# nzfeng/signed-heat-3d

Hardware: AMD Instinct MI355X
Metric: grid-nodes/sec end-to-end SHM (conv+PCG) (higher is better)
Workload: dtype f64 (Step 1: f64 / packed-f32 tiers)

## Files before the change

### signed-heat-3d_amd/csrc/shm_schur.hip.h

```cpp
#pragma once
#include "shm_kernels.hip.h"

namespace shm {

static __global__ __launch_bounds__(kBlock) void green_symbol_kernel(int n, const double* __restrict__ lam1, double* __restrict__ W0) {
    const double g0 = 0.5 / n, g1 = 1.0 / n;
    for (int row = blockIdx.x; row < n * n; row += gridDim.x) {
        const int k1 = row / n, k2 = row - k1 * n;
        const double l12 = lam1[k1] + lam1[k2];
        const double g12 = (k1 ? g1 : g0) * (k2 ? g1 : g0);
        double* const out = W0 + (size_t)row * n;
        for (int k3 = threadIdx.x; k3 < n; k3 += kBlock) {
            const double lam = l12 + lam1[k3];
            const double g = g12 * (k3 ? g1 : g0);
            out[k3] = (row | k3) ? g / lam : 0.;
        }
    }
}

static __global__ __launch_bounds__(kBlock) void cosine_tables_kernel(int n, int P, const double* __restrict__ ctab, double* __restrict__ Cm, double* __restrict__ Ct) {
    const int total = (n + 1) * n;
    for (int v = blockIdx.x * kBlock + threadIdx.x; v < total; v += gridDim.x * kBlock) {
        const int d = v / n, k = v - d * n;
        const double c = ctab[(int)(((long long)d * k) % (2 * n))];
        Cm[(size_t)d * n + k] = c;
        Ct[(size_t)k * P + d] = c;
    }
}

constexpr int kGemmT = 128, kGemmK = 16;
template <int WN>
__global__ __launch_bounds__(kBlock) __attribute__((amdgpu_waves_per_eu(WN == 4 ? 2 : WN == 2 ? 3 : 4, WN == 4 ? 2 : WN == 2 ? 3 : 4))) void dgemm_rm_kernel(int M, int N, int K, const double* __restrict__ A, int lda, long long sA, const double* __restrict__ B, int ldb,
                                                          long long sB, double* __restrict__ C, int ldc, long long sC, int prio) {
    constexpr int kTN = 32 * WN;
    if (prio) __builtin_amdgcn_s_setprio(3);
    __shared__ double as[kGemmT][kGemmK + 1];
    __shared__ double bs[kGemmK][kTN + 1];
    A += (long long)blockIdx.z * sA;
    B += (long long)blockIdx.z * sB;
    C += (long long)blockIdx.z * sC;
    const int i0 = blockIdx.y * kGemmT, j0 = blockIdx.x * kTN;
    const int lane = threadIdx.x & 63, w = threadIdx.x >> 6;
    const int wr = w >> 1, wc = w & 1;
    const int l15 = lane & 15, l4 = lane >> 4;
    gj_f64x4 acc[4][WN];
#pragma unroll
    for (int a = 0; a < 4; a++)
#pragma unroll
        for (int b = 0; b < WN; b++) acc[a][b] = gj_f64x4{0., 0., 0., 0.};
    constexpr int kPerA = kGemmT * kGemmK / kBlock, kPerB = kTN * kGemmK / kBlock;
    double ra[kPerA], rb[kPerB];
    auto fetch = [&](int kc) {
#pragma unroll
        for (int u = 0; u < kPerA; u++) {
            const int t = threadIdx.x + u * kBlock;
            const int k = t & (kGemmK - 1), i = t >> 4;
            ra[u] = (i0 + i < M && kc + k < K) ? A[(size_t)(i0 + i) * lda + kc + k] : 0.;
        }
#pragma unroll
        for (int u = 0; u < kPerB; u++) {
            const int t = threadIdx.x + u * kBlock;
            const int j = t & (kTN - 1), k2 = t / kTN;
            rb[u] = (kc + k2 < K && j0 + j < N) ? B[(size_t)(kc + k2) * ldb + j0 + j] : 0.;
        }
    };
    fetch(0);
    for (int kc = 0; kc < K; kc += kGemmK) {
        __syncthreads();
#pragma unroll
        for (int u = 0; u < kPerA; u++) {
            const int t = threadIdx.x + u * kBlock;
            as[t >> 4][t & (kGemmK - 1)] = ra[u];
        }
#pragma unroll
        for (int u = 0; u < kPerB; u++) {
            const int t = threadIdx.x + u * kBlock;
            bs[t / kTN][t & (kTN - 1)] = rb[u];
        }
        __syncthreads();
        if (kc + kGemmK < K) fetch(kc + kGemmK);
#pragma unroll
        for (int kk = 0; kk < kGemmK; kk += 4) {
            double af[4], bf[WN];
#pragma unroll
            for (int a = 0; a < 4; a++) af[a] = as[wr * 64 + a * 16 + l15][kk + l4];
#pragma unroll
            for (int b = 0; b < WN; b++) bf[b] = bs[kk + l4][wc * 16 * WN + b * 16 + l15];
#pragma unroll
            for (int a = 0; a < 4; a++)
#pragma unroll
                for (int b = 0; b < WN; b++) acc[a][b] = __builtin_amdgcn_mfma_f64_16x16x4f64(af[a], bf[b], acc[a][b], 0, 0, 0);
        }
    }
#pragma unroll
    for (int a = 0; a < 4; a++)
#pragma unroll
        for (int b = 0; b < WN; b++)
#pragma unroll
            for (int r = 0; r < 4; r++) {
                const int row = i0 + wr * 64 + a * 16 + l4 + 4 * r, col = j0 + wc * 16 * WN + b * 16 + l15;
                if (row < M && col < N) C[(size_t)row * ldc + col] = acc[a][b][r];
            }
}

__device__ __forceinline__ int schur_fold(int e, int n) { return e <= n ? e : 2 * n - e; }
typedef double schur_f64x2 __attribute__((ext_vector_type(2), aligned(8)));
static __global__ __launch_bounds__(kBlock) void schur_assemble_kernel(int m, int ld, int n, int P, const int* __restrict__ rowX ,
                                                                const double* __restrict__ rowT , const double* __restrict__ T, double* __restrict__ S, int prio) {
    if (blockIdx.x < blockIdx.y) return;
    if (prio) __builtin_amdgcn_s_setprio(3);
    const int i = blockIdx.y * 16 + (threadIdx.x >> 4), j = blockIdx.x * 16 + (threadIdx.x & 15);
    if (i >= m || j >= m || j < i) return;
    unsigned ox[2][3], oy[2][3], oz[2];
    double wx[2][3], wy[2][3], wz[2][3];
    const unsigned pitch_y = (unsigned)P, pitch_x = (unsigned)(n + 1) * (unsigned)P;
#pragma unroll
    for (int a = 0; a < 3; a++) {
        const int Xi = rowX[4 * i + a], Xj = rowX[4 * j + a];
        const double ti = rowT[3 * i + a], tj = rowT[3 * j + a];
        const double wi0 = 1. - ti, wi1 = ti, wj0 = 1. - tj, wj1 = tj;
        const int D = Xi - Xj, E = Xi + Xj + 1;
        const double wd[3] = {wi0 * wj1, wi0 * wj0 + wi1 * wj1, wi1 * wj0};
        const double ws[3] = {wi0 * wj0, wi0 * wj1 + wi1 * wj0, wi1 * wj1};
        int pd[3], ps[3];
#pragma unroll
        for (int e = 0; e < 3; e++) {
            pd[e] = abs(D - 1 + e);
            ps[e] = schur_fold(E + e, n);
        }
        if (a == 0) {
#pragma unroll
            for (int e = 0; e < 3; e++) {
                ox[0][e] = __umul24((unsigned)pd[e], pitch_x);
                ox[1][e] = __umul24((unsigned)ps[e], pitch_x);
                wx[0][e] = wd[e];
                wx[1][e] = ws[e];
            }
        } else if (a == 1) {
#pragma unroll
            for (int e = 0; e < 3; e++) {
                oy[0][e] = __umul24((unsigned)pd[e], pitch_y);
                oy[1][e] = __umul24((unsigned)ps[e], pitch_y);
                wy[0][e] = wd[e];
                wy[1][e] = ws[e];
            }
        } else {
#pragma unroll
            for (int f = 0; f < 2; f++) {
                const int* pz = f ? ps : pd;
                const double* wv = f ? ws : wd;
                const int zb = min(pz[0], min(pz[1], pz[2]));
                oz[f] = (unsigned)zb;
#pragma unroll
                for (int sl = 0; sl < 3; sl++) {
                    double w = 0.;
#pragma unroll
                    for (int e = 0; e < 3; e++) w += pz[e] - zb == sl ? wv[e] : 0.;
                    wz[f][sl] = w;
                }
            }
        }
    }
    double acc = 0.;
#pragma unroll
    for (int combo = 0; combo < 8; combo++) {
        const int fx = combo & 1, fy = (combo >> 1) & 1, fz = combo >> 2;
        const double* base = T + oz[fz];
        double sc = 0.;
#pragma unroll
        for (int p = 0; p < 3; p++) {
            double sp = 0.;
#pragma unroll
            for (int q = 0; q < 3; q++) {
                const double* row = base + (ox[fx][p] + oy[fy][q]);
                const schur_f64x2 lo = *reinterpret_cast<const schur_f64x2*>(row);
                const double hi = row[2];
                sp += wy[fy][q] * (wz[fz][0] * lo.x + wz[fz][1] * lo.y + wz[fz][2] * hi);
            }
            sc += wx[fx][p] * sp;
        }
        acc += sc;
    }
    const int ri = rowX[4 * i + 3], rj = rowX[4 * j + 3];
    S[(size_t)ri * ld + rj] = acc;
    S[(size_t)rj * ld + ri] = acc;
}

static __global__ __launch_bounds__(kBlock) void set_diagonal_kernel(double* __restrict__ M, int ld, int i0, int i1, double v) {
    const int i = i0 + blockIdx.x * kBlock + threadIdx.x;
    if (i < i1) M[(size_t)i * ld + i] = v;
}

static __global__ __launch_bounds__(kDualBlock) void dual_bordered_kernel(int m, const double* __restrict__ u, const double* __restrict__ v, const double* __restrict__ sigma_ptr,
                                                                  int accumulate, double* __restrict__ mu) {
    __shared__ double lds[17];
    double su = 0., sv = 0.;
    for (int a = threadIdx.x; a < m; a += kDualBlock) {
        su += u[a];
        sv += v[a];
    }
    su = block_sum_1024(su, lds);
    sv = block_sum_1024(sv, lds);
    const double c = (su - (sigma_ptr ? *sigma_ptr : 0.)) / sv;
    for (int a = threadIdx.x; a < m; a += kDualBlock) mu[a] = (accumulate ? mu[a] : 0.) + u[a] - c * v[a];
}

static __global__ __launch_bounds__(kBlock) void fill_kernel(double* __restrict__ x, int count, double v) {
    const int a = blockIdx.x * kBlock + threadIdx.x;
    if (a < count) x[a] = v;
}

}
```

### signed-heat-3d_amd/csrc/shm_solver.hip.h

```cpp
#pragma once
#include "shm_host.hip.h"
#include "shm_kernels.hip.h"
#include "shm_conv_tiered.hip.h"
#include "shm_cg_fused.hip.h"
#include "shm_twolevel.hip.h"
#include "shm_schur.hip.h"
#include "shm_dct.hip.h"
#include "shm_dct_gemm.hip.h"
#include "shm_green_fft.hip.h"
#include "shm_sample.hip.h"
#include "shm_audit.hip.h"
#include "shm_iso_indexed.hip.h"
#include "shm_plan.h"

namespace shm {

template <typename T> constexpr int vec_width() { return sizeof(T) == 8 ? 2 : 4; }

template <typename T>
struct Slab {
    int k0 = 0, k1 = 0, nzl = 0;
    size_t plane = 0, nown = 0, ntot = 0;
    DevArray<T> Y0, Y1, Y2, r , x, p, q , z ;
    DevArray<double> partials, pq_partials , red , pq , u , sc;
    DevArray<unsigned> proj_ticket;
    DevArray<int> row_ptr, ent_row, node_ptr;
    DevArray<uint32_t> ent_node, node_id;
    DevArray<double> ent_coef, nent_coef;
    DevArray<ShiftItem> shift_items;
    DevArray<double> dv;
    DevArray<int> layer_order;
    DevArray<int> sample_order;
    DevArray<unsigned char> sample_rule;
    DevArray<unsigned long long> sample_ctr;
    long long sample_key = -1;
    int sample_blocks = 0;
    long long layer_order_key = -1;
    DevArray<double> div_partials;
    int div_sum_blocks = 0;
    DevArray<T> touched_save;
    DevArray<T> W1, W2;
    DevArray<T> S1, S2, S4;
    DevArray<int> act_x, act_y;
    DevArray<unsigned> act_z;
    DevArray<int> act_planes;
    int n_act_planes = 0;
    int n_act_x = 0, n_act_y = 0;
    int n_touched = 0, n_shift = 0;
    GridParams gp{};
};

template <typename T>
struct Solver final : SolverBase {
    shm_config cfg;
    hipStream_t stream = nullptr;
    hipStream_t stream2 = nullptr;
    hipStream_t stream3 = nullptr;
    std::unique_ptr<Event> e_sch_in, e_sch_done, e_gs_done;
    hipStream_t stream_h = nullptr;
    int n = 0, alloc_n = -1;
    size_t N = 0;
    double cell = 0., lambda = 0.;
    double bbox_min[3] = {0, 0, 0};
    double conv_ctr[3] = {0, 0, 0};
    double conv_wscale = 1.;
    int64_t S = 0;
    std::vector<double> h_pos, h_wn, h_area;
    double area_sum = 0., conv_far_gap = 0., conv_skip_base = 3.0e38, last_host_setup_ms = 0., last_setup_wall_ms = 0.;
    double conv_tier_log = 0., conv_tier_skip_base = 3.0e38;
    double conv_drop_K = 64., conv_drop_eps64 = 2e-9, conv_drop_eps32 = 6.0e-8;
    double conv_w_span = 0.;
    DevArray<double> d_src_t;
    DevArray<float> d_clusters_t;
    int n_clusters_t = 0;
    bool conv_tiered = false;
    bool conv_tier_exact = false;
    bool conv_tiered32 = false;
    bool conv_reference = false;
    int step1_selected = SHM_STEP1_AUTO;
    int last_step1_arith = SHM_STEP1_AUTO;
    double last_step1_budget = 0.;
    bool fold_pq = false;
    int fold_pq_np = 0;
    double step1_budget = 0.;
    DevArray<unsigned long long> d_pair_counters;
    DevArray<unsigned> d_unit_counters;
    static constexpr int kMaxConvLaunches = 256;
    int conv_launch_index = 0;
    int conv_launches_last = 0;
    int n_clusters = 0;
    int conv_grid_cap = 1 << 30;
    bool o_fast_hint = false;
    int num_cus = 256;
    DevArray<T> d_src;
    DevArray<float> d_src32;
    DevArray<float> d_clusters;
    DevArray<double> d_exptab;
    std::vector<Slab<T>> slabs;
    int total_slabs = 1, first_slab = 0;
    std::vector<int32_t> slab_bounds;
    bool slabs_equal = true;
    void slab_range(int slab, int32_t* k0, int32_t* k1) const {
        *k0 = slab_bounds[(size_t)slab];
        *k1 = slab_bounds[(size_t)slab + 1];
    }
    bool have_problem = false, have_conv = false, have_div = false, have_phi = false, have_constraints = false;
    std::vector<Row> rows;
    std::vector<std::vector<ShiftItem>> shift_host;
    int m = 0, mp = 0;
    DevArray<double> Ginv, gjP, gjR, gjC;
    DevArray<float> Ginv32;
    struct TwoLevel {
        bool on = false;
        int box = 16, P = 0, nI = 0, nS = 0, nSp = 0, ysz = 0;
        DevArray<int> ptrI, ptrS, rowsI, colsS, sepRow, adj_ptr, adj_idx, colour_list, rowBox, chunkBox, chunkCol, tBox, tRow, sBox, sRow;
        DevArray<size_t> offW;
        DevArray<double> gjP, gjR, gjC;
        int nChunks = 0, nTChunks = 0, nbMax = 0;
        int schur_ptr[9] = {0, 0, 0, 0, 0, 0, 0, 0, 0};
        DevArray<size_t> offD, offE;
        DevArray<double> D, E, Tm, tbuf, ybuf, vS, uS;
        DevArray<float> D32, E32, T32;
        int colour_ptr[9] = {0, 0, 0, 0, 0, 0, 0, 0, 0};
        size_t szD = 0, szE = 0;
        TlBoxes view() const { return TlBoxes{ptrI.p, ptrS.p, offD.p, offE.p, rowsI.p, colsS.p}; }
    } tl;
    int ginv_rows = 0, ginv_ld = 0;
    DevArray<int> gjFlag;
    DevArray<double*> d_redptrs;
    DevArray<int> Bptr, Bcol;
    DevArray<double> Bval;
    bool have_B = false;
    using TP = T;
    DevArray<Cplx<TP>> d_tw, d_om;
    DevArray<TP> d_lam;
    DevArray<double> d_lam64;
    DevArray<double> gd_Cm, gd_Ct, gd_W1, gd_W2;
    DevArray<double> gs_lam, gs_ctab, gs_Cm, gs_Ct, gs_W0, gs_W1, gs_T, Sdense, d_rowT;
    DevArray<int> d_rowX;
    std::vector<double> h_gs_lam, h_gs_ctab, h_rowT;
    std::vector<Cplx<double>> h_gs_tw;
    DevArray<Cplx<double>> gs_tw;
    std::vector<int> h_rowX;
    bool have_S = false;
    DevArray<double> Sinv, Sinv_ones ;
    PlanIn plan_in;
    Plan plan;
    double conv_est_total_ms = 1e30;
    int log2n = 0;
    bool precond_ready = false;
    double* h_pinned = nullptr;
    Rccl::comm_t comm = nullptr;
    int vec = 1;
    std::unique_ptr<Solver<T>> full;
    bool solve_only = false;
    bool full_problem_set = false;
    bool pool_held = false;

    explicit Solver(const shm_config& c, bool solve_only_ = false) : cfg(c), solve_only(solve_only_) {
        int ndev = 0;
        hipError_t e = hipGetDeviceCount(&ndev);
        if (e != hipSuccess || ndev <= 0)
            throw Error(SHM_ERR_HIP, fmt("no HIP device available (%s); this library has no CPU fallback",
                                          e == hipSuccess ? "device count 0" : hipGetErrorString(e)));
        if (cfg.device < 0 || cfg.device >= ndev) throw Error(SHM_ERR_INVALID, fmt("device %d out of range [0,%d)", cfg.device, ndev));
        HIPCHK(hipSetDevice(cfg.device));
        HIPCHK(hipStreamCreateWithFlags(&stream, hipStreamNonBlocking));
        {
            hipDeviceProp_t prop;
            HIPCHK(hipGetDeviceProperties(&prop, cfg.device));
            conv_grid_cap = std::max(1, prop.multiProcessorCount * 4);
            num_cus = prop.multiProcessorCount;
        }
        {
            int least = 0, greatest = 0;
            HIPCHK(hipDeviceGetStreamPriorityRange(&least, &greatest));
            HIPCHK(hipStreamCreateWithPriority(&stream2, hipStreamNonBlocking, greatest));
        }
        HIPCHK(hipHostMalloc((void**)&h_pinned, 64 * sizeof(double)));
        if (cfg.world > 1 && !cfg.rccl_unique_id) throw Error(SHM_ERR_INVALID, "world>1 needs rccl_unique_id");
        if (cfg.rccl_unique_id) {
            Rccl& R = Rccl::get();
            Rccl::unique_id id;
            memcpy(&id, cfg.rccl_unique_id, sizeof id);
            R.chk(R.CommInitRank(&comm, cfg.world, id, cfg.rank), "ncclCommInitRank");
        }
        PinnedPool::get().acquire(cfg.device);
        pool_held = true;
    }
    ~Solver() override {
        (void)hipSetDevice(cfg.device);
        if (comm) (void)Rccl::get().CommDestroy(comm);
        if (h_pinned) (void)hipHostFree(h_pinned);
        for (void* b : smp_pinned)
            if (b) (void)hipHostFree(b);
        slabs.clear();
        if (stream) (void)hipStreamDestroy(stream);
        if (stream2) (void)hipStreamDestroy(stream2);
        if (stream3) (void)hipStreamDestroy(stream3);
        if (stream_h) (void)hipStreamDestroy(stream_h);
        if (pool_held) PinnedPool::get().release(cfg.device);
    }

    void log(const char* f, ...) {
        if (!cfg.verbose) return;
        va_list ap;
        va_start(ap, f);
        vfprintf(stderr, f, ap);
        va_end(ap);
        fputc('\n', stderr);
    }

    static int grid_for(size_t work_items, int cap = 2048) {
        size_t b = (work_items + kBlock - 1) / kBlock;
        if (b < 1) b = 1;
        if (b > (size_t)cap) b = cap;
        return (int)b;
    }

    void set_problem(const shm_sources& src, const shm_grid& g) override {
        HIPCHK(hipSetDevice(cfg.device));
        if (g.n < 2) throw Error(SHM_ERR_INVALID, "grid.n must be >= 2");
        if (!(g.cell > 0.) || !std::isfinite(g.cell)) throw Error(SHM_ERR_INVALID, "grid.cell must be positive and finite");
        if (src.S <= 0 || !src.pos || !src.wnormal || !src.area) throw Error(SHM_ERR_INVALID, "sources: S>0 and non-null arrays required");
        if (!(src.lambda > 0.) || !std::isfinite(src.lambda)) throw Error(SHM_ERR_INVALID, "sources.lambda must be positive and finite");
        if (src.S > (int64_t)1 << 28) throw Error(SHM_ERR_INVALID, "too many sources");
        total_slabs = cfg.world * cfg.local_slabs;
        first_slab = cfg.rank * cfg.local_slabs;
        if (g.n < total_slabs) throw Error(SHM_ERR_INVALID, fmt("grid.n=%d smaller than the number of z-slabs %d", g.n, total_slabs));
        n = g.n;
        N = (size_t)n * n * n;
        cell = g.cell;
        lambda = src.lambda;
        for (int a = 0; a < 3; a++) bbox_min[a] = g.bbox_min[a];
        S = src.S;
        h_pos.assign(src.pos, src.pos + 3 * S);
        h_wn.assign(src.wnormal, src.wnormal + 3 * S);
        h_area.assign(src.area, src.area + S);
        for (int64_t s = 0; s < S; s++)
            for (int a = 0; a < 3; a++) {
                const double d = (h_pos[3 * s + a] - bbox_min[a]) / cell;
                if (!(d >= 0.) || !(std::floor(d) + 1. <= (double)(n - 1)))
                    throw Error(SHM_ERR_INVALID, fmt("source %lld lies outside the grid cells", (long long)s));
            }
        area_sum = 0.;
        for (int64_t s = 0; s < S; s++) area_sum += h_area[s];
        {
            double lo[3] = {1e300, 1e300, 1e300}, hi[3] = {-1e300, -1e300, -1e300};
            for (int64_t s = 0; s < S; s++)
                for (int a = 0; a < 3; a++) {
                    lo[a] = std::min(lo[a], h_pos[3 * s + a]);
                    hi[a] = std::max(hi[a], h_pos[3 * s + a]);
                }
            const double ext = std::max({hi[0] - lo[0], hi[1] - lo[1], hi[2] - lo[2], 1e-300});
            auto spread = [](uint64_t v) {
                v &= 0x1fffff;
                v = (v | v << 32) & 0x1f00000000ffffULL;
                v = (v | v << 16) & 0x1f0000ff0000ffULL;
                v = (v | v << 8) & 0x100f00f00f00f00fULL;
                v = (v | v << 4) & 0x10c30c30c30c30c3ULL;
                v = (v | v << 2) & 0x1249249249249249ULL;
                return v;
            };
            std::vector<std::pair<uint64_t, int64_t>> order((size_t)S);
            for (int64_t s = 0; s < S; s++) {
                uint64_t code = 0;
                for (int a = 0; a < 3; a++) {
                    const uint64_t q = (uint64_t)std::min(1048575.0, std::max(0.0, (h_pos[3 * s + a] - lo[a]) / ext * 1048575.0));
                    code |= spread(q) << a;
                }
                order[(size_t)s] = {code, s};
            }
            std::sort(order.begin(), order.end());
            for (int a = 0; a < 3; a++) conv_ctr[a] = bbox_min[a] + 0.5 * (double)(n - 1) * cell;
            constexpr int kConvCluster = conv_cluster<T>();
            n_clusters = (int)((S + kConvCluster - 1) / kConvCluster);
            const int64_t Spad = (int64_t)n_clusters * kConvCluster;
            std::vector<T> packed((size_t)Spad * 6, (T)0);
            std::vector<float> packed32((size_t)Spad * 6, 0.f), cl((size_t)n_clusters * kConvClusterRec, 0.f);
            double amin = 1e300, amax = 0.;
            for (int64_t s = 0; s < S; s++) {
                const double w = std::sqrt(h_wn[3 * s] * h_wn[3 * s] + h_wn[3 * s + 1] * h_wn[3 * s + 1] + h_wn[3 * s + 2] * h_wn[3 * s + 2]);
                if (w > 0.) amin = std::min(amin, w);
                amax = std::max(amax, w);
            }
            conv_wscale = amax > 0. && std::isfinite(amax) ? std::ldexp(1.0, -std::ilogb(amax) - 1) : 1.0;
            conv_w_span = amax > 0. && amin < 1e300 ? std::log(amax / amin) : 0.;
            const double wscale = sizeof(T) == 4 ? conv_wscale : 1.0;
            for (int64_t t = 0; t < Spad; t++) {
                const int64_t s = order[(size_t)std::min<int64_t>(t, S - 1)].second;
                for (int a = 0; a < 3; a++) {
                    packed[6 * t + a] = (T)(h_pos[3 * s + a] - conv_ctr[a]);
                    packed32[6 * t + a] = (float)(h_pos[3 * s + a] - conv_ctr[a]);
                    if (t < S) {
                        packed[6 * t + 3 + a] = (T)(h_wn[3 * s + a] * wscale);
                        packed32[6 * t + 3 + a] = (float)(h_wn[3 * s + a] * wscale);
// ... 1217 lines not shown
            for (int k = 0; k <= nb; k++) {
                const size_t nU = k == 0 ? 0 : (k < nb ? (size_t)(nb - 1) * nb / 2 : (size_t)nb * (nb + 1) / 2);
                const unsigned grid = (unsigned)((k < nb ? nb : 0) + nU);
                double* Rn = gjR.p + (size_t)(k & 1) * kGJ * mp;
                double* Cn = gjC.p + (size_t)(k & 1) * mp * kGJ;
                const double* Rp = gjR.p + (size_t)((k + 1) & 1) * kGJ * mp;
                const double* Cp = gjC.p + (size_t)((k + 1) & 1) * mp * kGJ;
                hipLaunchKernelGGL(gj_step_kernel, dim3(grid), dim3(kBlock), 0, stream, M, mp, nb, k, Rp, Cp, Rn, Cn, gjFlag.p, plan.setup_prio);
            }
        } else if (outer == 1) {
            for (int kb = 0; kb < nb; kb++) {
                launch_pivot(kb);
                hipLaunchKernelGGL(gj_panels_kernel, dim3(nb), dim3(kBlock), 0, stream, M, mp, kb, gjP.p, gjR.p, 0, gjC.p, c_ld, 0, plan.setup_prio);
                hipLaunchKernelGGL((gj_update_kernel<GJ_ALL>), dim3((unsigned)((size_t)nb * (nb + 1) / 2)), dim3(kBlock), 0, stream, M, mp, nb, kb, 0, 1,
                                   gjR.p, 0, gjC.p, c_ld, 0, kGJ, plan.setup_prio);
            }
        } else {
            for (int k0 = 0; k0 < nb; k0 += outer) {
                const int nO = std::min(outer, nb - k0);
                for (int t = 0; t < nO; t++) {
                    const int kb = k0 + t;
                    launch_pivot(kb);
                    hipLaunchKernelGGL(gj_panels_kernel, dim3(nb), dim3(kBlock), 0, stream, M, mp, kb, gjP.p, gjR.p, t * kGJ, gjC.p, c_ld, t * kGJ, plan.setup_prio);
                    hipLaunchKernelGGL((gj_update_kernel<GJ_CROSS>), dim3((unsigned)(nO * nb + nO * k0)), dim3(kBlock), 0, stream, M, mp, nb, kb, k0, nO,
                                       gjR.p, t * kGJ, gjC.p, c_ld, t * kGJ, kGJ, plan.setup_prio);
                }
                const size_t nr = (size_t)(nb - nO);
                if (nr > 0)
                    hipLaunchKernelGGL((gj_update_kernel<GJ_REST>), dim3((unsigned)(nr * (nr + 1) / 2)), dim3(kBlock), 0, stream, M, mp, nb, -1, k0, nO,
                                       gjR.p, 0, gjC.p, c_ld, 0, nO * kGJ, plan.setup_prio);
            }
        }
        if (nb > 1) hipLaunchKernelGGL(gj_mirror_kernel, dim3((unsigned)((size_t)nb * (nb - 1) / 2)), dim3(kBlock), 0, stream, M, mp);
        HIPCHK(hipGetLastError());
    }
    void enqueue_invert_G() {
        const int mp = ginv_ld;
        enqueue_gj_invert(Ginv.p, mp);
        Ginv32.alloc((size_t)mp * mp);
        hipLaunchKernelGGL((convert_kernel<double, float>), dim3(grid_for((size_t)mp * mp, 4096)), dim3(kBlock), 0, stream2, (size_t)mp * mp, Ginv.p, Ginv32.p);
        HIPCHK(hipGetLastError());
    }
    void enqueue_green_table(hipStream_t st) {
        const int P = n + 8;
        const size_t n1 = (size_t)n + 1;
        {
            const double pi = 3.14159265358979323846;
            h_gs_lam.resize(n);
            h_gs_ctab.resize(2 * (size_t)n);
            for (int k = 0; k < n; k++) h_gs_lam[k] = (2. - 2. * std::cos(pi * k / n)) / (cell * cell);
            for (int r = 0; r < 2 * n; r++) h_gs_ctab[r] = std::cos(pi * r / n);
            gs_lam.upload(h_gs_lam, st);
            gs_ctab.upload(h_gs_ctab, st);
            gs_T.alloc(n1 * n1 * P);
        }
        {
            DevArray<double>&W0 = gs_W0, &W1 = gs_W1, &W2 = gs_W0;
            gs_Cm.alloc(n1 * n);
            gs_Ct.alloc((size_t)n * P);
            W0.alloc(std::max((size_t)n * n * n, (size_t)n * n1 * P));
            W1.alloc((size_t)n * n * P);
            const bool by_fft = (n & (n - 1)) == 0 && n >= 16 && n <= 512;
            if (by_fft) {
                const double pi = 3.14159265358979323846;
                h_gs_tw.resize(2 * (size_t)n);
                for (int t = 0; t < n; t++) {
                    h_gs_tw[(size_t)t] = {std::cos(2. * pi * t / n), -std::sin(2. * pi * t / n)};
                    h_gs_tw[(size_t)n + t] = {std::cos(pi * t / n), -std::sin(pi * t / n)};
                }
                gs_tw.upload(h_gs_tw, st);
                HIPCHK(hipMemsetAsync(W1.p, 0, (size_t)n * n * P * sizeof(double), st));
                hipLaunchKernelGGL(green_symbol_kernel, dim3((unsigned)std::min(n * n, 8 * num_cus)), dim3(kBlock), 0, st, n, gs_lam.p, W0.p);
                const long long Pl = P, n1l = (long long)n1;
                auto pass = [&](bool xpass, int ntiles, int tiles_a, DctAddr in, DctAddr out, const double* src, double* dst) {
                    CosiParams C;
                    C.ntiles = ntiles;
                    C.tiles_a = tiles_a;
                    C.in = in;
                    C.out = out;
                    const dim3 g((unsigned)std::min(ntiles, 16 * num_cus));
                    const Cplx<double>*tw = gs_tw.p, *om = gs_tw.p + n;
                    int l2 = 0;
                    while ((1 << l2) < n) l2++;
#define SHM_COSI_CASE(L)                                                                                                                              \
    case L:                                                                                                                                            \
        if (xpass) hipLaunchKernelGGL((cosi_lines_kernel<L, true>), g, dim3(kBlock), 0, st, C, src, dst, tw, om, plan.setup_prio);                         \
        else hipLaunchKernelGGL((cosi_lines_kernel<L, false>), g, dim3(kBlock), 0, st, C, src, dst, tw, om, plan.setup_prio);                              \
        break;
                    switch (l2) {
                        SHM_COSI_CASE(4) SHM_COSI_CASE(5) SHM_COSI_CASE(6) SHM_COSI_CASE(7) SHM_COSI_CASE(8) SHM_COSI_CASE(9)
                        default: throw Error(SHM_ERR_INVALID, "Green's table by FFT: n out of range");
                    }
#undef SHM_COSI_CASE
                };
                auto addr = [](long long a_stride, long long b_stride, long long line_stride, long long elem_stride) {
                    DctAddr A;
                    A.off = 0; A.a_stride = a_stride; A.b_stride = b_stride; A.line_stride = line_stride; A.elem_stride = elem_stride;
                    A.seg_stride = 0; A.seg_shift = 30; A.seg_mask = 0x3fffffff;
                    return A;
                };
                const int L = kCosiL;
                pass(true, n * n / L, n * n / L, addr((long long)L * n, 0, n, 1), addr((long long)L * Pl, 0, Pl, 1), W0.p, W1.p);
                pass(false, n * (P / L), P / L, addr(L, (long long)n * Pl, 1, Pl), addr(L, n1l * Pl, 1, Pl), W1.p, W2.p);
                pass(false, (int)(n1l * Pl / L), (int)(n1l * Pl / L), addr(L, 0, 1, n1l * Pl), addr(L, 0, 1, n1l * Pl), W2.p, gs_T.p);
                HIPCHK(hipGetLastError());
                return;
            }
            HIPCHK(hipMemsetAsync(gs_Ct.p, 0, (size_t)n * P * sizeof(double), st));
            hipLaunchKernelGGL(cosine_tables_kernel, dim3(grid_for(n1 * n, 1024)), dim3(kBlock), 0, st, n, P, gs_ctab.p, gs_Cm.p, gs_Ct.p);
            hipLaunchKernelGGL(green_symbol_kernel, dim3((unsigned)std::min(n * n, 8 * num_cus)), dim3(kBlock), 0, st, n, gs_lam.p, W0.p);
            const bool narrow = plan_in.tiered();
            auto tiles = [](size_t v) { return (unsigned)((v + kGemmT - 1) / kGemmT); };
            auto gemm = [&](unsigned batches, int M, int N, int K, const double* A, int lda, long long sA, const double* B, int ldb, long long sB, double* C, int ldc, long long sC) {
                if (narrow)
                    hipLaunchKernelGGL(dgemm_rm_kernel<1>, dim3((unsigned)((N + 31) / 32), tiles((size_t)M), batches), dim3(kBlock), 0, st, M, N, K, A, lda, sA, B, ldb, sB, C, ldc, sC, plan.setup_prio);
                else
                    hipLaunchKernelGGL(dgemm_rm_kernel<4>, dim3(tiles((size_t)N), tiles((size_t)M), batches), dim3(kBlock), 0, st, M, N, K, A, lda, sA, B, ldb, sB, C, ldc, sC, plan.setup_prio);
            };
            gemm(1, n * n, P, n, W0.p, n, 0LL, gs_Ct.p, P, 0LL, W1.p, P, 0LL);
            gemm((unsigned)n, (int)n1, P, n, gs_Cm.p, n, 0LL, W1.p, P, (long long)n * P, W2.p, P, (long long)(n1 * P));
            gemm(1, (int)n1, (int)(n1 * P), n, gs_Cm.p, n, 0LL, W2.p, (int)(n1 * P), 0LL, gs_T.p, (int)(n1 * P), 0LL);
            HIPCHK(hipGetLastError());
        }
    }
    void prepare_schur() {
        hipStream_t st = stream2;
        have_S = false;
        if (!plan.explicit_S) return;
        if (!plan.green_early) enqueue_green_table(st);
        std::vector<std::pair<uint64_t, int>> key((size_t)m);
        auto spread = [](uint64_t v) {
            v &= 0x1fffff;
            v = (v | v << 32) & 0x1f00000000ffffULL;
            v = (v | v << 16) & 0x1f0000ff0000ffULL;
            v = (v | v << 8) & 0x100f00f00f00f00fULL;
            v = (v | v << 4) & 0x10c30c30c30c30c3ULL;
            v = (v | v << 2) & 0x1249249249249249ULL;
            return v;
        };
        for (int r = 0; r < m; r++) key[(size_t)r] = {spread((uint64_t)rows[r].cell[0]) | spread((uint64_t)rows[r].cell[1]) << 1 | spread((uint64_t)rows[r].cell[2]) << 2, r};
        std::sort(key.begin(), key.end());
        h_rowX.resize(4 * (size_t)m);
        h_rowT.resize(3 * (size_t)m);
        for (int q = 0; q < m; q++) {
            const int r = key[(size_t)q].second;
            for (int a = 0; a < 3; a++) {
                h_rowX[4 * (size_t)q + a] = rows[r].cell[a];
                h_rowT[3 * (size_t)q + a] = rows[r].t[a];
            }
            h_rowX[4 * (size_t)q + 3] = r;
        }
        d_rowX.upload(h_rowX, st);
        d_rowT.upload(h_rowT, st);
        Sdense.alloc((size_t)mp * mp);
        if (!stream3) {
            int least = 0, greatest = 0;
            HIPCHK(hipDeviceGetStreamPriorityRange(&least, &greatest));
            HIPCHK(hipStreamCreateWithPriority(&stream3, hipStreamNonBlocking, greatest));
            e_sch_in.reset(new Event());
            e_sch_done.reset(new Event());
        }
        e_sch_in->record(st);
    }
    void enqueue_schur() {
        if (!plan.explicit_S) return;
        const bool dual_direct = plan.dual_form == SHM_DUAL_DIRECT;
        hipStream_t st = dual_direct ? stream2 : stream3;
        HIPCHK(hipStreamWaitEvent(st, e_sch_in->e, 0));
        const int P = n + 8;
        if (plan.green_early) HIPCHK(hipStreamWaitEvent(st, e_gs_done->e, 0));
        HIPCHK(hipMemsetAsync(Sdense.p, 0, (size_t)mp * mp * sizeof(double), st));
        const unsigned mt = (unsigned)((m + 15) / 16);
        hipLaunchKernelGGL(schur_assemble_kernel, dim3(mt, mt), dim3(kBlock), 0, st, m, mp, n, P, d_rowX.p, d_rowT.p, gs_T.p, Sdense.p, plan.setup_prio);
        HIPCHK(hipGetLastError());
        if (dual_direct) {
            Sinv.alloc((size_t)mp * mp);
            HIPCHK(hipMemcpyAsync(Sinv.p, Sdense.p, (size_t)mp * mp * sizeof(double), hipMemcpyDeviceToDevice, st));
            if (mp > m) hipLaunchKernelGGL(set_diagonal_kernel, dim3((unsigned)((mp - m + kBlock - 1) / kBlock)), dim3(kBlock), 0, st, Sinv.p, mp, m, mp, 1.0);
            enqueue_gj_invert(Sinv.p, mp, true);
            Sinv_ones.alloc((size_t)2 * mp);
            hipLaunchKernelGGL(fill_kernel, dim3((unsigned)((m + kBlock - 1) / kBlock)), dim3(kBlock), 0, st, Sinv_ones.p + mp, m, 1.0);
            launch_ginv_matvec<double>(st, m, m, mp, Sinv.p, Sinv_ones.p + mp, Sinv_ones.p);
        } else {
            e_sch_done->record(st);
            HIPCHK(hipStreamWaitEvent(stream2, e_sch_done->e, 0));
        }
        have_S = true;
    }
    void finish_invert_G() {
        hipStream_t stream = stream2;
        int flag[2] = {0, 0};
        if (!tl.on) HIPCHK(hipMemsetAsync(gjFlag.p + 1, 0, sizeof(int), stream));
        HIPCHK(hipMemcpyAsync(flag, gjFlag.p, 2 * sizeof(int), hipMemcpyDeviceToHost, stream));
        HIPCHK(hipStreamSynchronize(stream));
        if (flag[0] || flag[1]) throw Error(SHM_ERR_SINGULAR, "A A^T is not positive definite (duplicate or degenerate constraint rows)");
    }

    void allreduce(int which , int count) {
        auto buf = [&](Slab<T>& sl) { return which == 0 ? sl.red.p : sl.pq.p; };
        if (slabs.size() > 1) {
            double** slot = d_redptrs.p + (which ? slabs.size() : 0);
            hipLaunchKernelGGL(sum_slabs_kernel, dim3((count + kBlock - 1) / kBlock), dim3(kBlock), 0, stream, (int)slabs.size(), slot, count);
        }
        if (comm) {
            Rccl& R = Rccl::get();
            R.chk(R.AllReduce(buf(slabs[0]), buf(slabs[0]), (size_t)count, Rccl::kFloat64, Rccl::kSum, comm, stream), "ncclAllReduce");
            for (size_t s = 1; s < slabs.size(); s++)
                HIPCHK(hipMemcpyAsync(buf(slabs[s]), buf(slabs[0]), (size_t)count * sizeof(double), hipMemcpyDeviceToDevice, stream));
        }
    }

    void halo_exchange_p() { halo_exchange(ARR_P); }
    void halo_exchange(int sel) { halo_exchange(sel, stream); }
    void halo_exchange(int sel, hipStream_t stream) {
        const size_t pb = slabs[0].plane * sizeof(T);
        for (size_t s = 0; s + 1 < slabs.size(); s++) {
            Slab<T>&a = slabs[s], &b = slabs[s + 1];
            HIPCHK(hipMemcpyAsync(arr(b, sel), arr(a, sel) + (size_t)a.nzl * a.plane, pb, hipMemcpyDeviceToDevice, stream));
            HIPCHK(hipMemcpyAsync(arr(a, sel) + (size_t)(a.nzl + 1) * a.plane, arr(b, sel) + b.plane, pb, hipMemcpyDeviceToDevice, stream));
        }
        if (comm) {
            Rccl& R = Rccl::get();
            const int dt = sizeof(T) == 8 ? Rccl::kFloat64 : Rccl::kFloat32;
            Slab<T>&lo = slabs.front(), &hi = slabs.back();
            const size_t cnt = lo.plane;
            R.chk(R.GroupStart(), "ncclGroupStart");
            if (cfg.rank > 0) {
                R.chk(R.Send(arr(lo, sel) + lo.plane, cnt, dt, cfg.rank - 1, comm, stream), "ncclSend(lo)");
                R.chk(R.Recv(arr(lo, sel), cnt, dt, cfg.rank - 1, comm, stream), "ncclRecv(lo)");
            }
            if (cfg.rank < cfg.world - 1) {
                R.chk(R.Send(arr(hi, sel) + (size_t)hi.nzl * hi.plane, cnt, dt, cfg.rank + 1, comm, stream), "ncclSend(hi)");
                R.chk(R.Recv(arr(hi, sel) + (size_t)(hi.nzl + 1) * hi.plane, cnt, dt, cfg.rank + 1, comm, stream), "ncclRecv(hi)");
            }
            R.chk(R.GroupEnd(), "ncclGroupEnd");
        }
    }

    struct StencilLaunch {
        dim3 grid, block;
        int xchunks, yblocks, zc;
    };
    StencilLaunch stencil_dims(const Slab<T>& sl) const {
        const int per_row = (n + vec - 1) / vec;
        int tx = 1;
        while (tx < per_row && tx < kBlock) tx <<= 1;
        const int tyb = kBlock / tx;
        const int xchunks = (per_row + tx - 1) / tx;
        const int yblocks = (n + tyb * kStRY - 1) / (tyb * kStRY);
        int zc = 16;
        while (zc > 4 && (long long)xchunks * yblocks * ((sl.nzl + zc - 1) / zc) < 1024) zc >>= 1;
        const int zchunks = (sl.nzl + zc - 1) / zc;
        return {dim3((unsigned)(xchunks * yblocks * zchunks)), dim3((unsigned)tx, (unsigned)tyb), xchunks, yblocks, zc};
    }

    void launch_stencil(Slab<T>& sl) {
        const StencilLaunch L = stencil_dims(sl);
        if (vec == 1)
            hipLaunchKernelGGL((stencil_dot_kernel<T, 1>), L.grid, L.block, 0, stream, sl.gp, L.xchunks, L.yblocks, L.zc, sl.p.p, sl.q.p, sl.partials.p);
        else
            hipLaunchKernelGGL((stencil_dot_kernel<T, vec_width<T>()>), L.grid, L.block, 0, stream, sl.gp, L.xchunks, L.yblocks, L.zc, sl.p.p, sl.q.p, sl.partials.p);
    }

    template <int VEC> void launch_update_xr(Slab<T>& sl, int rho_slot, int grid) {
        hipLaunchKernelGGL((update_xr_kernel<T, VEC>), dim3(grid), dim3(kBlock), 0, stream, sl.nown / VEC, sl.plane, sl.sc.p, rho_slot, sl.pq.p,
                           sl.x.p, sl.p.p, sl.r.p, sl.q.p, sl.partials.p);
    }
    template <int VEC> void launch_update_p(Slab<T>& sl, int rho_old, int rho_new, int init, int use_uw, const T* zsrc, int grid) {
        hipLaunchKernelGGL((update_p_kernel<T, VEC>), dim3(grid), dim3(kBlock), 0, stream, sl.nown / VEC, sl.plane, sl.sc.p, rho_old, rho_new,
                           sl.red.p, init, use_uw, zsrc, sl.p.p);
    }
    void update_p_all(int rho_old, int rho_new, int init, bool pre, const std::vector<int>& nparts) {
        for (size_t s = 0; s < slabs.size(); s++) {
            const T* zsrc = pre ? slabs[s].z.p : slabs[s].r.p;
            if (vec == 1) launch_update_p<1>(slabs[s], rho_old, rho_new, init, pre ? 0 : 1, zsrc, nparts[s]);
            else launch_update_p<vec_width<T>()>(slabs[s], rho_old, rho_new, init, pre ? 0 : 1, zsrc, nparts[s]);
        }
    }
    template <int VEC> void launch_norm2(Slab<T>& sl, const T* v, int grid) {
        hipLaunchKernelGGL((norm2_kernel<T, VEC>), dim3(grid), dim3(kBlock), 0, stream, sl.nown / VEC, sl.plane, v, sl.partials.p);
    }

    struct FusedCfg {
        int wx = 0, ry = 8, zc = 16, yblocks = 0, zchunks = 0, nw = 8, part = 0;
    };
    bool fused_available() const {
        static const bool off = knob("SHM_CG_CLASSIC") != nullptr;
        return !off && (n + vec - 1) / vec <= 8 * 64;
    }
    FusedCfg fused_cfg(const Slab<T>& sl) const {
        FusedCfg c;
        const int lanes = (n + vec - 1) / vec;
        c.wx = 1;
        while (c.wx * 64 < lanes) c.wx <<= 1;
        static const int nw_env = knob("SHM_FUSED_WAVES") ? atoi(knob("SHM_FUSED_WAVES")) : 0;
        c.ry = (vec == 1) ? 4 : 2;
        c.nw = (c.ry <= 2 && (nw_env == 16 || (nw_env == 0 && c.wx >= 4))) ? 16 : 8;
        const int wy = c.nw / c.wx;
        static const int zc_env = knob("SHM_FUSED_ZC") ? atoi(knob("SHM_FUSED_ZC")) : 0;
        c.yblocks = (n + wy * c.ry - 1) / (wy * c.ry);
        const int want = std::max(1, (2 * num_cus + c.yblocks - 1) / c.yblocks);
        c.zc = std::min(64, std::max(8, sl.nzl / want));
        if (zc_env > 0) c.zc = zc_env;
        c.zc = std::max(1, std::min(c.zc, sl.nzl));
        c.zchunks = (sl.nzl + c.zc - 1) / c.zc;
        while ((size_t)c.yblocks * c.zchunks > sl.partials.count && c.zc < sl.nzl) {
            c.zc = std::min(sl.nzl, 2 * c.zc);
            c.zchunks = (sl.nzl + c.zc - 1) / c.zc;
        }
        return c;
    }
    enum FusedPart { FUSED_ALL = 0, FUSED_INTERIOR = 1, FUSED_BOUNDARY = 2 };
    template <int MODE, int VEC, int RY, int WX>
    void launch_fused_k(Slab<T>& sl, const FusedCfg& cc, int slot_old, int slot_new, int init, int use_uw, int alpha_slot, const T* zsrc, const T* pin, T* pout) {
        FusedCfg c = cc;
        FusedParams F;
        F.n = n; F.nzl = sl.nzl; F.k0 = sl.k0; F.zc = c.zc; F.yblocks = c.yblocks; F.inv_h2 = sl.gp.inv_h2;
        F.zc_first = 0; F.zc_stride = 1;
        const bool dir_to_own = fold_pq && MODE == CGF_DIR;
        const int pq_np = (fold_pq && MODE == CGF_RES) ? fold_pq_np : 0;
        if (fold_pq && !sl.pq_partials.p) sl.pq_partials.alloc(sl.partials.count);
        if (c.part == FUSED_INTERIOR) { F.zc_first = 1; c.zchunks -= 2; }
        else if (c.part == FUSED_BOUNDARY) { F.zc_stride = c.zchunks - 1; c.zchunks = 2; }
        if constexpr (RY <= 2) {
            if (c.nw == 16) {
                hipLaunchKernelGGL((cg_fused_kernel<T, VEC, RY, WX, 16 / WX, MODE>), dim3((unsigned)(c.yblocks * c.zchunks)), dim3(1024), 0, stream, F, sl.sc.p, slot_old,
                                   slot_new, sl.red.p, sl.pq.p, init, use_uw, alpha_slot, zsrc, pin, pout, sl.r.p, dir_to_own ? sl.pq_partials.p : sl.partials.p, sl.pq_partials.p, pq_np);
                return;
            }
        }
// ... 1543 lines not shown
```

Measured before the change: 673.6 million.

## Launch only upper-triangular Schur tiles in XCD-aware supertile order and dual-write S

Replaces the full mt×mt grid (half of which exited at once) with a compact list of upper-triangle tiles, grouped into 8×8 supertiles and remapped so each XCD gets a contiguous range, which should improve L2 reuse of the Green table. The full-matrix memset becomes a small kernel that clears only the padding rows and columns. In the dual-direct path the kernel writes S to both Sdense and Sinv, removing a full device-to-device copy. The cost is an extra tile-list upload and double scattered stores when the inverse is needed.

```diff
diff --git a/signed-heat-3d_amd/csrc/shm_schur.hip.h b/signed-heat-3d_amd/csrc/shm_schur.hip.h
--- a/signed-heat-3d_amd/csrc/shm_schur.hip.h
+++ b/signed-heat-3d_amd/csrc/shm_schur.hip.h
@@ -1,5 +1,6 @@
 #pragma once
 #include "shm_kernels.hip.h"
+#include "shm_tile_order.h"
 
 namespace shm {
 
@@ -106,10 +107,13 @@
 __device__ __forceinline__ int schur_fold(int e, int n) { return e <= n ? e : 2 * n - e; }
 typedef double schur_f64x2 __attribute__((ext_vector_type(2), aligned(8)));
 static __global__ __launch_bounds__(kBlock) void schur_assemble_kernel(int m, int ld, int n, int P, const int* __restrict__ rowX ,
-                                                                const double* __restrict__ rowT , const double* __restrict__ T, double* __restrict__ S, int prio) {
-    if (blockIdx.x < blockIdx.y) return;
+                                                                const double* __restrict__ rowT , const double* __restrict__ T, double* __restrict__ S, int prio,
+                                                                const uint32_t* __restrict__ tiles, unsigned ntiles, unsigned per, double* __restrict__ S2) {
+    const unsigned el = schur_element_of_block(blockIdx.x, per);
+    if (el >= ntiles) return;
     if (prio) __builtin_amdgcn_s_setprio(3);
-    const int i = blockIdx.y * 16 + (threadIdx.x >> 4), j = blockIdx.x * 16 + (threadIdx.x & 15);
+    const unsigned tile = tiles[el];
+    const int i = (int)(tile >> 16) * 16 + (threadIdx.x >> 4), j = (int)(tile & 0xffffu) * 16 + (threadIdx.x & 15);
     if (i >= m || j >= m || j < i) return;
     unsigned ox[2][3], oy[2][3], oz[2];
     double wx[2][3], wy[2][3], wz[2][3];
@@ -184,6 +188,22 @@
     const int ri = rowX[4 * i + 3], rj = rowX[4 * j + 3];
     S[(size_t)ri * ld + rj] = acc;
     S[(size_t)rj * ld + ri] = acc;
+    if (S2) {
+        S2[(size_t)ri * ld + rj] = acc;
+        S2[(size_t)rj * ld + ri] = acc;
+    }
+}
+
+static __global__ __launch_bounds__(kBlock) void clear_padding_kernel(double* __restrict__ M, double* __restrict__ M2, int ld, int m, int mp) {
+    const size_t v = (size_t)blockIdx.x * kBlock + threadIdx.x;
+    if (v >= (size_t)(mp - m) * mp) return;
+    const size_t r = (size_t)m + v / mp, c = v % mp;
+    M[r * ld + c] = 0.;
+    M[c * ld + r] = 0.;
+    if (M2) {
+        M2[r * ld + c] = 0.;
+        M2[c * ld + r] = 0.;
+    }
 }
 
 static __global__ __launch_bounds__(kBlock) void set_diagonal_kernel(double* __restrict__ M, int ld, int i0, int i1, double v) {
diff --git a/signed-heat-3d_amd/csrc/shm_solver.hip.h b/signed-heat-3d_amd/csrc/shm_solver.hip.h
--- a/signed-heat-3d_amd/csrc/shm_solver.hip.h
+++ b/signed-heat-3d_amd/csrc/shm_solver.hip.h
@@ -142,6 +142,9 @@
     std::vector<Cplx<double>> h_gs_tw;
     DevArray<Cplx<double>> gs_tw;
     std::vector<int> h_rowX;
+    std::vector<uint32_t> h_schurTiles;
+    DevArray<uint32_t> d_schurTiles;
+    int schur_tiles_mt = -1;
     bool have_S = false;
     DevArray<double> Sinv, Sinv_ones ;
     PlanIn plan_in;
@@ -1665,6 +1668,12 @@
         }
         d_rowX.upload(h_rowX, st);
         d_rowT.upload(h_rowT, st);
+        const int mt = (m + 15) / 16;
+        if (mt != schur_tiles_mt) {
+            h_schurTiles = schur_tile_sequence(mt);
+            d_schurTiles.upload(h_schurTiles, st);
+            schur_tiles_mt = mt;
+        }
         Sdense.alloc((size_t)mp * mp);
         if (!stream3) {
             int least = 0, greatest = 0;
@@ -1682,13 +1691,14 @@
         HIPCHK(hipStreamWaitEvent(st, e_sch_in->e, 0));
         const int P = n + 8;
         if (plan.green_early) HIPCHK(hipStreamWaitEvent(st, e_gs_done->e, 0));
-        HIPCHK(hipMemsetAsync(Sdense.p, 0, (size_t)mp * mp * sizeof(double), st));
-        const unsigned mt = (unsigned)((m + 15) / 16);
-        hipLaunchKernelGGL(schur_assemble_kernel, dim3(mt, mt), dim3(kBlock), 0, st, m, mp, n, P, d_rowX.p, d_rowT.p, gs_T.p, Sdense.p, plan.setup_prio);
+        if (dual_direct) Sinv.alloc((size_t)mp * mp);
+        double* const S2 = dual_direct ? Sinv.p : nullptr;
+        if (mp > m) hipLaunchKernelGGL(clear_padding_kernel, dim3((unsigned)(((size_t)(mp - m) * mp + kBlock - 1) / kBlock)), dim3(kBlock), 0, st, Sdense.p, S2, mp, m, mp);
+        const size_t ntiles = h_schurTiles.size();
+        hipLaunchKernelGGL(schur_assemble_kernel, dim3(schur_grid(ntiles)), dim3(kBlock), 0, st, m, mp, n, P, d_rowX.p, d_rowT.p, gs_T.p, Sdense.p, plan.setup_prio,
+                           d_schurTiles.p, (unsigned)ntiles, (unsigned)schur_tiles_per_range(ntiles), S2);
         HIPCHK(hipGetLastError());
         if (dual_direct) {
-            Sinv.alloc((size_t)mp * mp);
-            HIPCHK(hipMemcpyAsync(Sinv.p, Sdense.p, (size_t)mp * mp * sizeof(double), hipMemcpyDeviceToDevice, st));
             if (mp > m) hipLaunchKernelGGL(set_diagonal_kernel, dim3((unsigned)((mp - m + kBlock - 1) / kBlock)), dim3(kBlock), 0, st, Sinv.p, mp, m, mp, 1.0);
             enqueue_gj_invert(Sinv.p, mp, true);
             Sinv_ones.alloc((size_t)2 * mp);
diff --git a/signed-heat-3d_amd/csrc/shm_tile_order.h b/signed-heat-3d_amd/csrc/shm_tile_order.h
--- /dev/null
+++ b/signed-heat-3d_amd/csrc/shm_tile_order.h
@@ -0,0 +1,27 @@
+#pragma once
+#include <cstdint>
+#include <vector>
+
+namespace shm {
+
+constexpr int kSchurXcds = 8;
+constexpr int kSchurSuper = 8;
+
+inline std::vector<uint32_t> schur_tile_sequence(int mt, int B = kSchurSuper) {
+    std::vector<uint32_t> seq;
+    seq.reserve((size_t)mt * (mt + 1) / 2);
+    for (int I = 0; I < mt; I += B)
+        for (int J = I; J < mt; J += B)
+            for (int ti = I; ti < I + B && ti < mt; ti++)
+                for (int tj = J > ti ? J : ti; tj < J + B && tj < mt; tj++) seq.push_back((uint32_t)ti << 16 | (uint32_t)tj);
+    return seq;
+}
+
+inline int schur_tiles_per_range(size_t tiles) { return (int)((tiles + kSchurXcds - 1) / kSchurXcds); }
+inline unsigned schur_grid(size_t tiles) { return (unsigned)(kSchurXcds * schur_tiles_per_range(tiles)); }
+#if defined(__HIPCC__)
+__host__ __device__
+#endif
+inline unsigned schur_element_of_block(unsigned b, unsigned per) { return (b % kSchurXcds) * per + b / kSchurXcds; }
+
+}
```

Result: no change. 673.0 million, median of 2 (-0.1%).
